# KyleVanMeter/MVOLPS

Hardware: AMD Instinct MI355X
Metric: simplex_pivots_per_s (higher is better)
Workload: dtype f64

## Files before the change

mvolps_amd/csrc/engine.cpp:

```cpp
#include <hip/hip_runtime.h>

#include <cmath>
#include <cstdio>
#include <cstdlib>
#include <cstring>
#include <atomic>
#include <map>
#include <mutex>
#include <tuple>
#include <unordered_map>
#include <vector>

#include "engine.hpp"

struct DevMatrix {
  int m0 = 0, n = 0, lda = 0;
  double *plain = nullptr, *packed = nullptr;
  int *len = nullptr;
  std::vector<const void *> rows;
  ~DevMatrix() {
    if (packed && packed != plain) (void)hipFree(packed);
    if (plain) (void)hipFree(plain);
    if (len) (void)hipFree(len);
  }
// ... 727 lines not shown
    P->nflag[j] = sflag ? sflag[j] : std_flag(P->ctype[j]);
    nlb[j] = P->clb[j];
    nub[j] = P->cub[j];
    xn[j] = nb_value(P->nflag[j], nlb[j], nub[j]);
    any_x = any_x || xn[j] != 0.0;
  }
  for (int i = 1; i <= m; i++) {
    P->bvar[i] = i;
    blb[i] = P->rlb[i];
    bub[i] = P->rub[i];
  }
  const size_t rows_per_chunk = std::max<size_t>(1, ((size_t)32 << 20) / ((size_t)ld * 8));
  double *bounce = nullptr;
  HIPCHECK(hipHostMalloc((void **)&bounce, rows_per_chunk * ld * 8));
  for (size_t r0 = 0; r0 <= (size_t)m; r0 += rows_per_chunk) {
    size_t r1 = std::min<size_t>((size_t)m + 1, r0 + rows_per_chunk);
    for (size_t i = r0; i < r1; i++) {
      double *row = bounce + (i - r0) * ld;
      std::memset(row, 0, (size_t)ld * 8);
      if (i == 0) {
        double z = P->c[0];
        for (int j = 1; j <= n; j++) {
          row[j] = P->c[j];
          if (xn[j] != 0.0) z = std::fma(P->c[j], xn[j], z);
        }
        row[0] = z;
      } else {
        const double *a = P->A[i]->data();
        std::memcpy(row + 1, a + 1, (size_t)n * 8);
        double acc = 0.0;
        if (any_x)
          for (int j = 1; j <= n; j++)
            if (xn[j] != 0.0) acc = std::fma(a[j], xn[j], acc);
        row[0] = acc;
      }
    }
    HIPCHECK(hipMemcpyAsync(P->d_T + r0 * ld, bounce, (r1 - r0) * ld * 8, hipMemcpyHostToDevice, sc.stream));
    HIPCHECK(hipStreamSynchronize(sc.stream));
  }
  HIPCHECK(hipHostFree(bounce));
  HIPCHECK(hipMemcpyAsync(P->d_bvar, P->bvar.data(), (size_t)(m + 1) * 4, hipMemcpyHostToDevice, sc.stream));
  HIPCHECK(hipMemcpyAsync(P->d_blb, blb.data(), (size_t)(m + 1) * 8, hipMemcpyHostToDevice, sc.stream));
  HIPCHECK(hipMemcpyAsync(P->d_bub, bub.data(), (size_t)(m + 1) * 8, hipMemcpyHostToDevice, sc.stream));
  std::vector<int> nv((size_t)ld, 0), nf((size_t)ld, MVX_NS);
  for (int j = 1; j <= n; j++) {
    nv[j] = P->nvar[j];
    nf[j] = P->nflag[j];
  }
  HIPCHECK(hipMemcpyAsync(P->d_nvar, nv.data(), (size_t)ld * 4, hipMemcpyHostToDevice, sc.stream));
  HIPCHECK(hipMemcpyAsync(P->d_nflag, nf.data(), (size_t)ld * 4, hipMemcpyHostToDevice, sc.stream));
  HIPCHECK(hipMemcpyAsync(P->d_nlb, nlb.data(), (size_t)ld * 8, hipMemcpyHostToDevice, sc.stream));
  HIPCHECK(hipMemcpyAsync(P->d_nub, nub.data(), (size_t)ld * 8, hipMemcpyHostToDevice, sc.stream));
  HIPCHECK(hipStreamSynchronize(sc.stream));
  rebuild_pos(P);
  P->pending.clear();
  P->valid = true;
  P->sol_fresh = false;
  P->fresh_rows = -1;
  P->status = MVX_UNDEF;
  return true;
}

static void flush_update_events(Context &c, size_t used) {
  for (size_t k = 0; k + 1 < used; k += 2) {
    float ms = 0.f;
    HIPCHECK(hipEventElapsedTime(&ms, c.ev_pool[k], c.ev_pool[k + 1]));
    c.prof_update_ms += ms;
    c.prof_update_n++;
  }
}

constexpr int PERSIST_HEAD_STRIDE_MAX = 4;
static std::atomic<int> g_persist_mode{-1};
static std::atomic<bool> g_persist_broken{false};
static std::atomic<long long> g_persist_launches{0}, g_persist_aborts{0};
struct PersistPlan {
  int cpw = 0, nw = 0;
  size_t lds = 0;
};
static bool persist_plan(Context &c, const mvx_prob *P, PersistPlan *pl) {
  if (g_persist_broken) return false;
  if (g_persist_mode < 0) {
    const char *e = std::getenv("MVX_PERSIST");
    g_persist_mode = (e && e[0] == '0') ? 0 : ((e && e[0] == '2') ? 2 : 1);
  }
  if (!g_persist_mode) return false;
  static int cus = 0;
  if (!cus) {
    hipDeviceProp_t prop;
    if (hipGetDeviceProperties(&prop, c.dev) != hipSuccess) return false;
    cus = prop.multiProcessorCount;
  }
  const int m = P->m, n = P->n;
  if ((long)(m + 1) * (n + 1) < 32768) return false;
  if (g_persist_mode < 2 && (long)(m + 1) * (n + 1) > 700000) return false;
  const int cpw = (n + cus - 1) / cus;
  if (cpw > persist_max_cpw()) return false;
  pl->cpw = cpw;
  pl->nw = (n + cpw - 1) / cpw;
  if (pl->nw > 256) return false;
  pl->lds = persist_lds_bytes(m, cpw);
  return pl->lds <= (size_t)150 * 1024;
}

static bool ensure_persist(Context &c, SolveCtx &sc, const mvx_prob *P, const PersistPlan &pl) {
  const int words = persist_slot_words(P->m_cap);
  if (!sc.d_pabort) {
    HIPCHECK(hipMalloc((void **)&sc.d_pabort, 1024));
    HIPCHECK(hipMemsetAsync(sc.d_pabort, 0, 1024, sc.stream));
    HIPCHECK(hipHostMalloc((void **)&sc.h_pabort, 1024));
    sc.h_pabort[0] = 0;
    HIPCHECK(hipMalloc((void **)&sc.d_pcand, (size_t)2 * 256 * PERSIST_HEAD_STRIDE_MAX * 8));
    HIPCHECK(hipMalloc((void **)&sc.d_pctl, sizeof(Ctl)));
  }
  if (words > sc.p_msg_words) {
    HIPCHECK(hipStreamSynchronize(sc.stream));
    if (sc.d_pmsg) HIPCHECK(hipFree(sc.d_pmsg));
    HIPCHECK(hipMalloc((void **)&sc.d_pmsg, (size_t)2 * 256 * words * 8));
    sc.p_msg_words = words;
  }
  if (P->ld > sc.p_pw_ld) {
    HIPCHECK(hipStreamSynchronize(sc.stream));
    if (sc.d_ppw) HIPCHECK(hipFree(sc.d_ppw));
    HIPCHECK(hipMalloc((void **)&sc.d_ppw, (size_t)2 * P->ld * 8));
    sc.p_pw_ld = P->ld;
  }
  if (sc.p_backup_bytes != P->slab_bytes) {
    if (sc.p_backup) slab_recycle(c, sc.p_backup, sc.p_backup_bytes);
    sc.p_backup = slab_alloc(c, P->slab_bytes);
    sc.p_backup_bytes = sc.p_backup ? P->slab_bytes : 0;
    if (!sc.p_backup) {
      (void)g_last_error.exchange(0);
      return false;
    }
  }
  (void)pl;
  return true;
}

struct SolveJob {
  mvx_prob *P = nullptr;
  SolveCtx *sc = nullptr;
  mvx_smcp parm;
  enum { MAIN, PHASE1, FINAL } mode = MAIN;
  int batch = 8, pb = 4;
  int done = D_RUN;
  bool try_fused = false;
  bool try_dfused = false;
  bool persist_queued = false;
  int seen_steps = 0, seen_pivots = 0, seen_bulk = 0;
  int chain = 1, chain0 = 1;
  bool resident = false;
  bool cluster = false;
  ChainArgs cargs{};
  size_t ev_used = 0;
  bool profiled = false;
  int rc = 0;
  Ctl snap;
};

static int pivot_budget(const mvx_prob *P, const mvx_smcp &parm) {
  return parm.it_lim >= 0 ? parm.it_lim : 200 * (P->m + P->n) + 100000;
}

static void stage_copy_async(SolveCtx &sc, const mvx_prob *P) {
  HIPCHECK(hipEventRecord(sc.ev_b, sc.stream));
  if (!sc.stage_zc) HIPCHECK(hipMemcpyAsync(sc.h_stage, sc.d_stage, stage_size(P->m_cap, P->ld), hipMemcpyDeviceToHost, sc.stream));
  if (sc.d_pabort) HIPCHECK(hipMemcpyAsync(sc.h_pabort, sc.d_pabort, 512, hipMemcpyDeviceToHost, sc.stream));
}

static bool dual_fused_worth_it(const mvx_prob *P) {
  static int mode = -1;
  if (mode < 0) {
    const char *e = std::getenv("MVX_DUAL_FUSED");
    mode = e ? std::atoi(e) : 1;
  }
  if (mode == 0) return false;
  if (mode >= 2) return true;
  const long entries = (long)(P->m + 1) * (P->n + 1);
  return entries >= 2000000 && entries < 12000000;
}

static void job_begin(Context &c, SolveJob &J) {
  mvx_prob *P = J.P;
  SolveCtx &sc = *J.sc;
  ensure_scratch(sc, P->m_cap, P->ld);
  Ctl *h = sc.h_ctl;
  fill_ctl(sc, P, h);
  h->tol_bnd = J.parm.tol_bnd;
  h->tol_dj = J.parm.tol_dj;
  h->tol_piv = J.parm.tol_piv;
  h->budget = pivot_budget(P, J.parm);
  take_edits(P, h);
  upload_ctl(sc);
  HIPCHECK(hipEventRecord(sc.ev_a, sc.stream));
  {
    ChainArgs &a = J.cargs;
    a.c = sc.d_ctl;
    a.T = P->d_T;
    a.blb = P->d_blb; a.bub = P->d_bub; a.nlb = P->d_nlb; a.nub = P->d_nub; a.nflag = P->d_nflag;
    a.betab = sc.d_betab;
    for (int k = 0; k < 2; k++) {
      a.pw[k] = sc.d_pw[k];
      a.drowk[k] = sc.d_drowk[k]; a.pwk[k] = sc.d_pwk[k]; a.nlbk[k] = sc.d_nlbk[k]; a.nubk[k] = sc.d_nubk[k]; a.nflagk[k] = sc.d_nflagk[k];
      a.betak[k] = sc.d_betak[k]; a.blbk[k] = sc.d_blbk[k]; a.bubk[k] = sc.d_bubk[k];
    }
    a.pp = sc.d_ppart; a.rp = sc.d_rpart; a.ppstride = sc.pp_stride; a.rpstride = sc.rp_stride;
    a.srow0 = sc.d_srowk[0]; a.colq0 = sc.d_colqk[0];
    a.sstride = sc.sk_stride; a.cstride = sc.ck_stride;
    a.m = P->m; a.n = P->n; a.ld = P->ld; a.mcap1 = P->m_cap + 1;
    a.ncb = chain_ncb(P->n); a.nrb = chain_nrb(P->m);
    a.tol_dj = h->tol_dj; a.tol_piv = h->tol_piv; a.tol_bnd = h->tol_bnd; a.sgn = h->sgn;
    a.stall_limit = h->stall_limit;
    a.zeros = sc.d_zeros;
    a.xg = sc.d_xg; a.xg_bytes = (int)XG_BYTES; a.xabort = sc.d_xabort;
    a.nw = chain_cluster_nw(P->m, P->n); a.kmax = 0; a.tagbase = 0; a.boot = 0;
  }
  J.cluster = J.resident && cluster_wanted() && chain_cluster_kmax(P->m, P->n) > 0;
  J.try_fused = !P->hint_dual;
  J.chain = J.chain0 = h->chain_max;
  J.try_dfused = P->hint_dual && dual_fused_worth_it(P);
  J.profiled = c.prof && J.sc == &c.main;
  if (J.parm.it_lim > 8 && J.try_fused) J.batch = std::min(J.parm.it_lim, 256);
}

static void job_enqueue(Context &c, SolveJob &J) {
  mvx_prob *P = J.P;
  SolveCtx &sc = *J.sc;
  const int m = P->m, n = P->n;
  J.ev_used = 0;
  if (J.mode == SolveJob::FINAL) {
    launch_export(sc.d_ctl, sc.d_stage, m, n, 1, sc.stream);
    stage_copy_async(sc, P);
    return;
  }
  if (J.mode == SolveJob::PHASE1) {
    for (int k = 0; k < J.pb; k++) {
      launch_p1_head(sc.d_ctl, sc.stream);
      launch_p1_fix(sc.d_ctl, n, sc.stream);
      launch_p1_select(sc.d_ctl, sc.stream);
      launch_update(sc.d_ctl, m + 1, n, sc.stream);
    }
    launch_export(sc.d_ctl, sc.d_stage, m, n, 0, sc.stream);
    stage_copy_async(sc, P);
    return;
  }
  const int batch = J.batch;
  if (J.profiled && c.ev_pool.size() < (size_t)2 * batch + 4) {
    size_t old = c.ev_pool.size();
    c.ev_pool.resize((size_t)2 * batch + 4);
    for (size_t k = old; k < c.ev_pool.size(); k++) HIPCHECK(hipEventCreate(&c.ev_pool[k]));
  }
  const int remaining = (J.parm.it_lim >= 0) ? std::max(0, J.parm.it_lim - J.seen_pivots) : (1 << 30);
  auto ev = [&]() {
    if (J.profiled) HIPCHECK(hipEventRecord(c.ev_pool[J.ev_used++], sc.stream));
  };
  int depth;
  if (J.try_fused) depth = std::max(0, std::min(batch, remaining));
  else depth = std::max(1, std::min(batch, remaining));
  auto body = [&](int m_grid) {
    if (J.try_fused) {
      PersistPlan pl;
      if (depth > 0 && !J.profiled && J.resident && !(J.cluster && !g_cluster_broken.load()) && persist_plan(c, P, &pl) && ensure_persist(c, sc, P, pl)) {
        launch_select(sc.d_ctl, sc.stream);
        launch_update(sc.d_ctl, m_grid, n, sc.stream, 1, 1);
        HIPCHECK(hipMemcpyAsync(sc.p_backup, P->slab, P->slab_bytes, hipMemcpyDeviceToDevice, sc.stream));
        HIPCHECK(hipMemcpyAsync(sc.d_pctl, sc.d_ctl, sizeof(Ctl), hipMemcpyDeviceToDevice, sc.stream));
        HIPCHECK(hipMemcpyAsync(sc.d_ppw, sc.d_pw[0], (size_t)P->ld * 8, hipMemcpyDeviceToDevice, sc.stream));
        HIPCHECK(hipMemcpyAsync(sc.d_ppw + P->ld, sc.d_pw[1], (size_t)P->ld * 8, hipMemcpyDeviceToDevice, sc.stream));
        const int head_stride = 4;
        HIPCHECK(hipMemsetAsync(sc.d_pcand, 0, (size_t)2 * pl.nw * head_stride * 8, sc.stream));
        const int steps = 1 << 24;
        if (launch_persist(sc.d_ctl, sc.d_pcand, sc.d_pmsg, sc.d_pabort, (unsigned long long *)(sc.d_pabort + 16), P->m, pl.cpw, pl.nw, sc.p_msg_words, steps, head_stride, sc.stream) == 0) {
          J.persist_queued = true;
          g_persist_launches++;
          launch_select(sc.d_ctl, sc.stream);
          launch_update(sc.d_ctl, m_grid, n, sc.stream, 1, 1);
        } else {
          g_persist_broken = true;
        }
      } else {
        const size_t e_generic = J.ev_used;
        if (J.profiled) J.ev_used += 2;
        if (depth > 0) {
          const bool cl = J.cluster && !g_cluster_broken.load();
          if (!cl) launch_pboot(J.cargs, sc.stream);
          bool first = true;
          const int kc = cl ? std::max(1, std::min(J.chain0, chain_cluster_kmax(m, n))) : std::max(1, J.chain);
          auto chain_launch = [&](int steps) {
            J.cargs.kmax = steps;
            J.cargs.boot = first ? 1 : 0;
            first = false;
            J.cargs.tagbase = sc.xtag;
            sc.xtag += 128;
            if (launch_chain(J.cargs, sc.stream) != 0) g_cluster_broken.store(true);
            g_cluster_launches++;
          };
          for (int left = depth; left > 0;) {
            const int steps = std::min(kc, left);
            if (cl) chain_launch(steps);
            else
              for (int t = 0; t < steps; t++) launch_pstep(J.cargs, t, sc.stream);
            ev();
            launch_fbc3(J.cargs, steps, sc.stream);
            ev();
            launch_fpatch(J.cargs, steps, sc.stream);
            left -= steps;
          }
          if (J.parm.it_lim >= 0 && depth >= remaining && !cl) launch_pc(J.cargs, 0, sc.stream);
        }
        launch_select(sc.d_ctl, sc.stream);
        if (J.profiled) HIPCHECK(hipEventRecord(c.ev_pool[e_generic], sc.stream));
        launch_update(sc.d_ctl, m_grid, n, sc.stream, 1, 1);
        if (J.profiled) HIPCHECK(hipEventRecord(c.ev_pool[e_generic + 1], sc.stream));
      }
    } else if (J.try_dfused) {
      launch_select(sc.d_ctl, sc.stream);
      launch_update(sc.d_ctl, m_grid, n, sc.stream, 1, 1);
      if (depth > 1) {
        launch_dboot(sc.d_ctl, n, sc.stream);
        launch_db(sc.d_ctl, m_grid, n, sc.stream);
        for (int k = 0; k < depth - 1; k++) {
          launch_da(sc.d_ctl, n, sc.stream);
          launch_db(sc.d_ctl, m_grid, n, sc.stream);
        }
      }
    } else {
      for (int k = 0; k < depth; k++) {
        launch_dsel(sc.d_ctl, m, n, sc.stream);
        launch_select(sc.d_ctl, sc.stream);
        ev();
        launch_update(sc.d_ctl, m_grid, n, sc.stream, 1, 1);
        ev();
      }
    }
    launch_export(sc.d_ctl, sc.d_stage, m_grid, n, 0, sc.stream);
    stage_copy_async(sc, P);
  };
  body(m);
}

static bool job_finalize(SolveJob &J) {
  mvx_prob *P = J.P;
  SolveCtx &sc = *J.sc;
  const Ctl &snap = J.snap;
  const unsigned char *s = sc.h_stage;
  const double *beta = (const double *)(s + sizeof(Ctl));
  const double *dj = beta + (P->m_cap + 1);
  const int *bv = (const int *)(dj + P->ld);
  const int *nv = bv + (P->m_cap + 1);
  const int *nf = nv + P->ld;
  P->beta.assign(beta, beta + P->m + 1);
  P->dj.assign(dj, dj + P->n + 1);
  P->bvar.assign(bv, bv + P->m + 1);
  P->nvar.assign(nv, nv + P->n + 1);
  P->nflag.assign(nf, nf + P->n + 1);
  rebuild_pos(P);
  P->sol_fresh = true;
  P->fresh_rows = -1;
  float ms = 0.f;
  HIPCHECK(hipEventElapsedTime(&ms, sc.ev_a, sc.ev_b));
  P->last_ms = ms;
  P->it_cnt += snap.it_cnt;
  P->bland_cnt += snap.n_bland;
  P->pert_cnt += snap.n_pert;
  P->hint_dual = false;
  switch (J.done) {
    case D_OPT: P->status = MVX_OPT; J.rc = 0; break;
    case D_UNBND: P->status = MVX_UNBND; J.rc = 0; break;
    case D_NOFEAS: P->status = MVX_NOFEAS; J.rc = 0; break;
    case D_ITLIM:
      P->status = (snap.phase == PH_PRIMAL2) ? MVX_FEAS : MVX_INFEAS;
      J.rc = MVX_EITLIM;
      break;
    default: P->status = MVX_UNDEF; J.rc = MVX_EFAIL; break;
  }
  return true;
}

static bool job_collect(Context &c, SolveJob &J) {
  SolveCtx &sc = *J.sc;
  Ctl &snap = J.snap;
  if (J.persist_queued) {
    J.persist_queued = false;
    if (sc.h_pabort[0]) {
      mvx_prob *P = J.P;
      g_persist_broken = true;
      g_persist_aborts++;
      std::fprintf(stderr, "mvx: resident-tableau launch aborted (workgroups not co-resident in time); using the two-kernel path from now on\n");
      HIPCHECK(hipMemcpyAsync(P->slab, sc.p_backup, P->slab_bytes, hipMemcpyDeviceToDevice, sc.stream));
      HIPCHECK(hipMemcpyAsync(sc.d_ctl, sc.d_pctl, sizeof(Ctl), hipMemcpyDeviceToDevice, sc.stream));
      HIPCHECK(hipMemcpyAsync(sc.d_pw[0], sc.d_ppw, (size_t)P->ld * 8, hipMemcpyDeviceToDevice, sc.stream));
      HIPCHECK(hipMemcpyAsync(sc.d_pw[1], sc.d_ppw + P->ld, (size_t)P->ld * 8, hipMemcpyDeviceToDevice, sc.stream));
      HIPCHECK(hipMemsetAsync(sc.d_pabort, 0, sizeof(int), sc.stream));
      sc.h_pabort[0] = 0;
      J.try_fused = true;
      return false;
    }
  }
  std::memcpy(&snap, sc.h_stage, sizeof(Ctl));
  if (J.mode == SolveJob::FINAL) return job_finalize(J);
  if (J.mode == SolveJob::PHASE1) {
    if (snap.done == D_RUN) {
      J.pb = std::min(J.pb * 2, 64);
      return false;
    }
    if (snap.done == D_PFEAS) {
      snap.rounds++;
      if (snap.rounds >= 64) {
        J.done = D_FAIL;
        J.mode = SolveJob::FINAL;
        return false;
      }
      snap.done = D_RUN;
      snap.phase = PH_START;
      *sc.h_ctl = snap;
      upload_ctl(sc);
      J.mode = SolveJob::MAIN;
      J.batch = 8;
      J.try_fused = false;
      J.try_dfused = false;
      return false;
    }
    J.done = snap.done;
    return job_finalize(J);
  }
  if (J.profiled) {
    const int steps_now = snap.n_bulk;
    flush_update_events(c, std::min(J.ev_used, (size_t)2 * (size_t)(steps_now - J.seen_steps)));
    J.seen_steps = steps_now;
  }
  if (snap.cl_abort) {
    g_cluster_broken.store(true);
    g_cluster_aborts++;
    std::fprintf(stderr, "mvx: cluster selection launch aborted (peer workgroups not reachable in time); using two launches per chained step from now on\n");
    HIPCHECK(hipMemsetAsync(sc.d_xabort, 0, sizeof(int), sc.stream));
  }
  J.done = snap.done;
  {
    const int dp = snap.it_cnt - J.seen_pivots, db = snap.n_bulk - J.seen_bulk;
    if (J.chain0 > 1 && db >= 4) {
      if (2 * dp < J.chain * db) J.chain = std::max(1, J.chain / 2);
      else if (10 * dp >= 9 * J.chain * db) J.chain = std::min(J.chain0, J.chain * 2);
    }
    J.seen_bulk = snap.n_bulk;
  }
  J.seen_pivots = snap.it_cnt;
  J.try_fused = (snap.phase == PH_PRIMAL2) && snap.stall < snap.stall_limit;
  J.try_dfused = (snap.phase == PH_DUAL) && snap.stall < snap.stall_limit && dual_fused_worth_it(J.P);
  if (J.done == D_NEED_PHASE1) {
    snap.done = D_RUN;
    snap.phase = PH_PHASE1;
    snap.p1_init = 1;
    snap.p1_fix_q = 0;
    *sc.h_ctl = snap;
    upload_ctl(sc);
    J.mode = SolveJob::PHASE1;
    J.pb = 4;
    return false;
  }
  if (J.done != D_RUN) return job_finalize(J);
  J.batch = std::min(J.batch * 2, 256);
  return false;
}

static bool already_solved(const mvx_prob *P, const mvx_smcp &parm) {
  if (!P->valid || parm.it_lim == 0) return false;
  if (P->status != MVX_OPT) return false;
  return P->last_tol[0] == parm.tol_bnd && P->last_tol[1] == parm.tol_dj && P->last_tol[2] == parm.tol_piv;
}
static void remember_tolerances(mvx_prob *P, const mvx_smcp &parm) {
  P->last_tol[0] = parm.tol_bnd;
  P->last_tol[1] = parm.tol_dj;
  P->last_tol[2] = parm.tol_piv;
}

static bool job_prepare(SolveJob &J, mvx_prob *P, const mvx_smcp *parm) {
  J.P = P;
  if (parm) J.parm = *parm;
  else mvx_init_smcp(&J.parm);
  if (P->m < 1 || P->n < 1) {
    P->status = MVX_UNDEF;
    J.rc = MVX_EFAIL;
    return false;
  }
  if (already_solved(P, J.parm)) {
    P->last_ms = 0.0;
    J.rc = 0;
    return false;
  }
  if (!P->valid && !build_slack_tableau(P)) {
    J.rc = MVX_EFAIL;
    return false;
  }
  remember_tolerances(P, J.parm);
  return true;
}

static int solve_once(mvx_prob *P, const mvx_smcp *parm, bool aux) {
  SolveJob J;
  if (!job_prepare(J, P, parm)) return J.rc;
  P->fresh_rows = -1;
  Context &c = ctx();
  HIPCHECK(hipSetDevice(c.dev));
  std::unique_lock<std::recursive_mutex> main_lock(c.main_mu);
  flush_copies(c);
  if (aux) main_lock.unlock();
  std::unique_lock<std::mutex> aux_lock(c.aux_mu, std::defer_lock);
  if (aux) aux_lock.lock();
  if (aux && !c.aux_ready) {
    init_solve_ctx(c.aux);
    c.aux_ready = true;
  }
  J.sc = aux ? &c.aux : &c.main;
  static std::atomic<bool> g_resident_token{false};
  bool expected = false;
  J.resident = g_resident_token.compare_exchange_strong(expected, true);
  job_begin(c, J);
  for (;;) {
    job_enqueue(c, J);
    HIPCHECK(hipStreamSynchronize(J.sc->stream));
    if (job_collect(c, J)) break;
  }
  if (J.resident) g_resident_token.store(false);
  return J.rc;
}

static int g_check_every = 1024;
static double g_refresh_tol = 1e-9;
void set_refresh(int check_every, double tol) {
  g_check_every = check_every > 0 ? check_every : 1024;
  g_refresh_tol = tol >= 0.0 ? tol : 1e-9;
}

constexpr int REFRESH_SAMPLE_ROWS = 32;
static double row_residual_sample(const mvx_prob *P, int rows);
double row_residual(const mvx_prob *P) { return row_residual_sample(P, 0); }

static double row_residual_sample(const mvx_prob *P, int rows) {
  if (!P->valid) return 0.0;
  refresh_solution(P);
  const int m = P->m, n = P->n;
  auto value = [&](int k) {
    const int pos = P->pos[(size_t)k];
    if (pos > 0) return P->beta[(size_t)pos];
    double lb, ub;
    var_bounds(P, k, &lb, &ub);
    return nb_value(P->nflag[(size_t)-pos], lb, ub);
  };
  std::vector<double> x((size_t)n + 1, 0.0);
  for (int j = 1; j <= n; j++) x[(size_t)j] = value(m + j);
  double worst = 0.0;
  const bool all = rows <= 0 || rows >= m;
  const int cnt = all ? m : rows;
  for (int k = 0; k < cnt; k++) {
    const int i = all ? k + 1 : 1 + (int)(((unsigned)P->it_cnt * 2654435761u + (unsigned)k * 0x9E3779B1u) % (unsigned)m);
    const double *a = P->A[(size_t)i]->data();
    double acc = 0.0;
    for (int j = 1; j <= n; j++) acc = acc + a[j] * x[(size_t)j];
    const double xr = value(i);
    const double r = std::fabs(acc - xr) / (1.0 + std::fabs(xr));
    if (r > worst) worst = r;
  }
  return worst;
}

static bool refresh_tableau(mvx_prob *P) {
  Context &c = ctx();
  MAIN_LOCK(c);
  flush_copies(c);
  SolveCtx &sc = c.main;
  const int m = P->m, n = P->n;
  std::vector<int> tflag((size_t)m + n + 1, 0), sflag((size_t)n + 1, 0);
  for (int j = 1; j <= n; j++) tflag[(size_t)P->nvar[(size_t)j]] = P->nflag[(size_t)j];
  for (int j = 1; j <= n; j++) sflag[(size_t)j] = tflag[(size_t)m + j] ? tflag[(size_t)m + j] : std_flag(P->ctype[(size_t)j]);
  const int status = P->status;
  if (!build_slack_tableau(P, sflag.data())) return false;
  ensure_scratch(sc, P->m_cap, P->ld);
  HIPCHECK(hipMemcpyAsync(sc.d_tflag, tflag.data(), tflag.size() * 4, hipMemcpyHostToDevice, sc.stream));
  fill_ctl(sc, P, sc.h_ctl);
  upload_ctl(sc);
  for (int k = m + 1; k <= m + n; k++) {
    if (tflag[(size_t)k]) continue;
    launch_refresh_select(sc.d_ctl, sc.d_tflag, k, sc.stream);
    launch_update(sc.d_ctl, m, n, sc.stream);
// ... 942 lines not shown
```

mvolps_amd/csrc/kernels.hip:

```cpp
#include <hip/hip_runtime.h>

#include <cmath>
#include <cstdlib>

#include "mvx_internal.hpp"

namespace mvx {

#define TIDX ((int)threadIdx.x)

__device__ __forceinline__ double xdiv(double a, double b) {
  const double q = a / b;
  const double aq = fabs(q);
  if (!(aq > 1e-290 && aq < 1e290)) return q;
  const double r = fma(-q, b, a);
  if (r == 0.0) return q;
  const bool up = (r > 0.0) == (b > 0.0);
  long long bits = __double_as_longlong(q);
  bits += ((q > 0.0) == up) ? 1 : -1;
  const double q1 = __longlong_as_double(bits);
  const double r1 = fma(-q1, b, a);
  return (fabs(r1) < fabs(r)) ? q1 : q;
}

// ... 2048 lines not shown
    tf = ubq - lbq;
    if (p == 0 || tf <= tstep) flip = true;
  }
  if (!flip && p == 0) {
    if (lead && g == 0) c->fstate = F_STOP;
    return;
  }
  PR_STAMP(1);
  const int pr = flip ? 1 : p;
  const double val0 = T[(size_t)pr * ld + jc];
  const double piv = A.colq0[(size_t)g * A.cstride + pr];
  const double bp = (g == 0) ? A.betab[pr] : A.betak[xr][pr];
  const double plb = (g == 0) ? A.blb[pr] : A.blbk[xr][pr], pub = (g == 0) ? A.bub[pr] : A.bubk[xr][pr];
  const double rcp = A.colq0[(size_t)rl * A.cstride + pr];
  rec.ip = xdiv(1.0, rec.piv);
  const double rcd = xdiv(rcp, rec.piv);
  PR_STAMP(2);
  double sj = 0.0, dnew, wnew;
  int fnew, kind, lf = 0, stall_new;
  double delta = 0.0, bound = 0.0, s0 = 0.0, xq = 0.0;
  if (flip) {
    const int nf = (sdir > 0) ? MVX_NU : MVX_NL;
    delta = (sdir > 0) ? tf : -tf;
    kind = ST_FLIP;
    lf = nf;
    dnew = (j == 0) ? fma(dq, delta, dj) : dj;
    wnew = wj;
    fnew = (j == q) ? nf : fj;
    stall_new = 0;
  } else {
    double val = val0;
#define PR_ROWSTEP(S, TV)                                                                              \
  if ((S) < g) {                                                                                       \
    const int lk = rl_i(rec.kind, (S));                                                                \
    if (lk == ST_PIVOT) {                                                                              \
      const int lp = rl_i(rec.p, (S)), lq = rl_i(rec.q, (S));                                          \
      if (lp == p) val = (j == lq) ? rl_d(rec.ip, (S)) : -(TV);                                        \
      else val = (j == lq) ? rl_d(rcd, (S)) : fma(-rl_d(rcp, (S)), (TV), val);                         \
    }                                                                                                  \
  }
#pragma unroll
    for (int s = 0; s < 16; s++) { PR_ROWSTEP(s, ta[s]) }
    if (g > 16) {
#pragma unroll
      for (int s = 0; s < 16; s++) { PR_ROWSTEP(16 + s, tb[s]) }
    }
#undef PR_ROWSTEP
    bound = p_up ? pub : plb;
    lf = dev_leave_flag(plb, pub, p_up);
    s0 = xdiv(bp - bound, piv);
    sj = (j == 0) ? s0 : xdiv(val, piv);
    dnew = (j == q) ? xdiv(dq, piv) : fma(-dq, sj, dj);
    if (j == q) {
      const double cc = xdiv(wq, piv * piv);
      wnew = cc > 1.0 ? cc : 1.0;
      lbj = plb;
      ubj = pub;
    } else {
      const double cc = sj * sj * wq;
      wnew = cc > wj ? cc : wj;
    }
    fnew = (j == q) ? lf : fj;
    kind = ST_PIVOT;
    xq = dev_nb_value(fq, lbq, ubq);
    stall_new = (tstep <= DEGEN_TOL) ? stall + 1 : 0;
  }
  if (!act || j == 0) fnew = MVX_NS;
  PR_STAMP(3);
  Cand best{0.0, 0.0, 0, 0};
  if (fnew != MVX_NS) {
    Cand x{0.0, 0.0, 0, 0};
    if (price_col(fnew, A.sgn * dnew, A.tol_dj, j, wnew, x)) best = x;
  }
  publish_pricing(A, best, b, dnew, wnew, lbj, ubj, fnew, s_slots, s_pay);
  PR_STAMP(4);
  if (act) {
    A.srow0[(size_t)g * A.sstride + j] = sj;
    A.drowk[xw][j] = dnew;
    A.pwk[xw][j] = (j >= 1) ? wnew : 1.0;
    A.nflagk[xw][j] = (j >= 1) ? fnew : MVX_NS;
    A.nlbk[xw][j] = lbj;
    A.nubk[xw][j] = ubj;
  }
  if (lead) {
    c->ch_kind[g] = kind;
    c->ch_p[g] = flip ? 0 : p;
    c->ch_q[g] = q;
    c->ch_lf[g] = lf;
    c->ch_piv[g] = flip ? 1.0 : piv;
    c->ch_xq[g] = xq;
    c->ch_s0[g] = s0;
    c->ch_delta[g] = delta;
    c->ch_elb[g] = lbq;
    c->ch_eub[g] = ubq;
    c->ch_llb[g] = plb;
    c->ch_lub[g] = pub;
    c->ch_bound[g] = bound;
    c->ch_pup[g] = p_up;
    c->ch_stall[g] = stall_new;
    c->ch_cnt[g] = used + (flip ? 0 : 1);
    c->ch_ok[g] = epoch;
    c->pc_n = g + 1;
  }
  PR_STAMP(5);
#undef PR_STAMP
}

constexpr int XNW = 64;
constexpr int XNF = 8;
enum : int { XAUX_SC0 = 1, XAUX_SC1 = 16 };
typedef unsigned xu4 __attribute__((ext_vector_type(4)));

struct XCtx {
  __amdgpu_buffer_rsrc_t rs;
  int w, nw;
  unsigned tag;
  int xno;
  int *xabort;
  bool dead;
  bool flag;
};

__device__ __forceinline__ double ld_sc1(const double *p) {
  return __longlong_as_double((long long)__hip_atomic_load(reinterpret_cast<const unsigned long long *>(p), __ATOMIC_RELAXED, __HIP_MEMORY_SCOPE_AGENT));
}

template <int MODE, int NP>
__device__ __forceinline__ Cand xchg(XCtx &X, Cand mine, const double (&pin)[NP], double (&pout)[NP], Cand (*s_slots)[4], double (*s_pay)[4][5]) {
  const int lane = TIDX & 63, wave = TIDX >> 6, b = X.xno & 1;
  int ol;
  Cand wb = wave_argbest<MODE>(mine, &ol);
  wb.aux = (wb.aux & 0xffff) | (__ballot(X.flag) ? 0x10000 : 0);
  if (lane == 0) s_slots[b][wave] = wb;
#pragma unroll
  for (int k = 0; k < NP; k++) {
    const double v = rl_d(pin[k], ol);
    if (lane == 0) s_pay[b][wave][k] = v;
  }
  __syncthreads();
  Cand bb = s_slots[b][0];
  int bw = 0, fl = bb.aux & 0x10000;
#pragma unroll
  for (int k = 1; k < 4; k++) {
    const Cand y = s_slots[b][k];
    fl |= y.aux & 0x10000;
    if (cand_better<MODE>(y, bb)) {
      bb = y;
      bw = k;
    }
  }
  bb.aux = (bb.aux & 0xffff) | fl;
  const unsigned tag = X.tag;
  const unsigned reg = (unsigned)(X.xno & 3) * (unsigned)(XNF * XNW * 16);
  if (TIDX < 3 + NP) {
    double v;
    if (TIDX == 0) v = bb.k1;
    else if (TIDX == 1) v = bb.k2;
    else if (TIDX == 2) v = __hiloint2double(bb.aux, bb.idx);
    else v = s_pay[b][bw][TIDX - 3];
    const xu4 x = {(unsigned)__double2loint(v), tag, (unsigned)__double2hiint(v), tag};
    __builtin_amdgcn_raw_buffer_store_b128(x, X.rs, reg + (unsigned)(TIDX * XNW + X.w) * 16, 0, XAUX_SC0);
  }
  double rec[3 + NP];
  const int lr = lane < X.nw ? lane : 0;
  unsigned spins = 0;
  for (;;) {
    bool ok = true;
#pragma unroll
    for (int f = 0; f < 3 + NP; f++) {
      const xu4 x = __builtin_amdgcn_raw_buffer_load_b128(X.rs, reg + (unsigned)(f * XNW + lr) * 16, 0, XAUX_SC1);
      ok &= (x.y == tag) & (x.w == tag);
      rec[f] = __hiloint2double((int)x.z, (int)x.x);
    }
    if (__all(ok)) break;
    ++spins;
    if ((spins & 255u) == 0) {
      if (spins > 2000000u) __hip_atomic_store(X.xabort, 1, __ATOMIC_RELAXED, __HIP_MEMORY_SCOPE_AGENT);
      if (spins > 2000000u || __hip_atomic_load(X.xabort, __ATOMIC_RELAXED, __HIP_MEMORY_SCOPE_AGENT)) {
        X.dead = true;
        break;
      }
    }
    __builtin_amdgcn_s_sleep(1);
  }
  X.tag++;
  X.xno++;
  Cand rc{0.0, 0.0, 0, 0};
  if (lane < X.nw && !X.dead) rc = Cand{rec[0], rec[1], __double2loint(rec[2]), __double2hiint(rec[2])};
  int wl;
  Cand win = wave_argbest<MODE>(rc, &wl);
  X.flag = __ballot((rc.aux & 0x10000) != 0) != 0ull;
  win.aux = (int)(short)(win.aux & 0xffff);
#pragma unroll
  for (int k = 0; k < NP; k++) pout[k] = rl_d(rec[3 + k], wl);
  return win;
}

template <int CPT, int RPT>
__global__ __launch_bounds__(256) void k_chain(const ChainArgs A) {
  extern __shared__ double hist[];
  __shared__ Cand s_slots[2][4];
  __shared__ double s_pay[2][4][5];
  __shared__ int s_kind[KCH], s_p[KCH], s_q[KCH];
  __shared__ double s_piv[KCH], s_ip[KCH], s_wv[4][2][KCH];
  if (blockIdx.x & 7) return;
  const int w = (int)blockIdx.x >> 3, t = TIDX, lane = t & 63, wave = t >> 6;
  Ctl *const c = A.c;
  const int nw = A.nw, TT = nw * 256, gt = w * 256 + t;
  const int m = A.m, n = A.n, kmax = A.kmax;
  const size_t ld = (size_t)A.ld;
  const double *const T = A.T;
  const bool lead = (gt == 0);
  unsigned long long *const dbg = c->dbg;
#define CH_STAMP(K) do { if (dbg && lead) dbg[(size_t)g * 16 + (K)] = __builtin_amdgcn_s_memrealtime(); } while (0)
  const int done = c->done, fstate0 = c->fstate, budget = c->budget, perturbed = c->perturbed, aborted = c->cl_abort, epoch = c->pc_epoch;
  const int phase0 = c->phase, n_edits = c->n_edits, cur0 = c->curA & 1;
  int stall = c->stall;
  const bool boot = (A.boot != 0);
  const bool fresh = boot && (phase0 == PH_START);
  const int fstate = boot ? F_RUN : fstate0;
  const bool boot_off = boot && (stall >= A.stall_limit || !(phase0 == PH_PRIMAL2 || (fresh && n_edits == 0)));
  double d[CPT], wgt[CPT], lbj[CPT], ubj[CPT], sqn[CPT];
  int f[CPT], jj[CPT];
#pragma unroll
  for (int u = 0; u < CPT; u++) {
    const int j = 1 + gt + u * TT;
    const bool act = (j <= n);
    const int jc = act ? j : n;
    jj[u] = j;
    d[u] = T[jc];
    wgt[u] = fresh ? 1.0 : A.pw[boot ? cur0 : 0][jc];
    f[u] = act ? A.nflag[jc] : MVX_NS;
    lbj[u] = A.nlb[jc];
    ubj[u] = A.nub[jc];
    sqn[u] = 0.0;
  }
  double z = T[0];
  double be[RPT], lb[RPT], ub[RPT];
  int ii[RPT];
#pragma unroll
  for (int u = 0; u < RPT; u++) {
    const int i = 1 + gt + u * TT;
    const int ic = (i <= m) ? i : m;
    ii[u] = i;
    be[u] = boot ? T[(size_t)ic * ld] : A.betab[ic];
    lb[u] = A.blb[ic];
    ub[u] = A.bub[ic];
  }
  if (done != D_RUN || fstate != F_RUN || aborted) return;
  if (boot_off) {
    if (lead) c->fstate = F_OFF;
    return;
  }
  XCtx X;
  X.rs = __builtin_amdgcn_make_buffer_rsrc(A.xg, 0, A.xg_bytes, 0x00027000);
  X.w = w;
  X.nw = nw;
  X.tag = A.tagbase + 1;
  X.xno = 0;
  X.xabort = A.xabort;
  X.dead = false;
  X.flag = false;
  if (fresh) {
    const double tolb = A.tol_bnd;
#pragma unroll
    for (int u = 0; u < RPT; u++) {
      if (ii[u] <= m) {
        if (lb[u] > -INFINITY && be[u] < lb[u] - tolb * (1.0 + fabs(lb[u]))) X.flag = true;
        if (ub[u] < INFINITY && be[u] > ub[u] + tolb * (1.0 + fabs(ub[u]))) X.flag = true;
      }
    }
  }
#define HS(S, U) hist[((size_t)(S) * (CPT + RPT) + (U)) * 256 + t]
#define HC(S, U) hist[((size_t)(S) * (CPT + RPT) + CPT + (U)) * 256 + t]
  int g = 0, used = 0;
  Cand pc;
  double pp[5], po[5];
#define PRICE()                                                                                          \
  do {                                                                                                   \
    pc = Cand{0.0, 0.0, 0, 0};                                                                           \
    pp[0] = d[0]; pp[1] = wgt[0]; pp[2] = lbj[0]; pp[3] = ubj[0]; pp[4] = sqn[0];                        \
    _Pragma("unroll") for (int u = 0; u < CPT; u++) {                                                    \
      Cand x{0.0, 0.0, 0, 0};                                                                            \
      if (f[u] != MVX_NS && price_col(f[u], A.sgn * d[u], A.tol_dj, jj[u], wgt[u], x) && cand_better<0>(x, pc)) { \
        pc = x;                                                                                          \
        pc.aux = (x.aux > 0 ? 1 : 0) | (f[u] << 1);                                                      \
        pp[0] = d[u]; pp[1] = wgt[u]; pp[2] = lbj[u]; pp[3] = ubj[u]; pp[4] = sqn[u];                    \
      }                                                                                                  \
    }                                                                                                    \
  } while (0)
  PRICE();
  Cand qc = xchg<0, 5>(X, pc, pp, po, s_slots, s_pay);
  if (boot && !X.dead) {
    if (X.flag) {
      if (lead) c->fstate = F_OFF;
      return;
    }
    if (lead) {
      c->fstate = F_RUN;
      c->step = ST_NONE;
    }
  }
  X.flag = false;
  bool end_itlim = false;
  for (;;) {
    if (X.dead) break;
    const int q = qc.idx;
    const bool none = (q == 0);
    const int left = (budget < 0) ? 1 : budget - used;
    if (none || left <= 0 || stall >= A.stall_limit) {
      const bool itlim = (!none && left <= 0 && stall < A.stall_limit && !perturbed);
      if (g == 0) {
        if (lead) {
          c->fstate = F_STOP;
          c->phase = PH_PRIMAL2;
          if (itlim) {
            c->done = D_ITLIM;
            c->step = ST_NONE;
          }
        }
      } else
        end_itlim = itlim;
      break;
    }
    if (g >= kmax) break;
    CH_STAMP(0);
    const int sdir = (qc.aux & 1) ? 1 : -1, fq = qc.aux >> 1;
    const double dq = po[0], wq = po[1], lbq = po[2], ubq = po[3];
    double a[RPT];
#pragma unroll
    for (int u = 0; u < RPT; u++) a[u] = T[(size_t)((ii[u] <= m) ? ii[u] : m) * ld + q];
    {
      double sqv = po[4];
      if (lane < g - 1) sqv = ld_sc1(A.srow0 + (size_t)lane * A.sstride + q);
      if (lane < g) s_wv[wave][0][lane] = sqv;
    }
    const int gu = __builtin_amdgcn_readfirstlane(g);
    const bool ispc = (lane < gu) && (s_kind[lane < KCH ? lane : 0] == ST_PIVOT);
    const unsigned pivm = (unsigned)__ballot(ispc);
    const unsigned spc = (unsigned)__ballot(ispc && s_q[lane < KCH ? lane : 0] == q);
    {
      int s0 = 0;
#define COL_BLOCK(N)                                                                                                     \
  if (gu - s0 >= N) {                                                                                                    \
    const unsigned bm = ((1u << N) - 1u) << s0;                                                                          \
    double hc8[RPT][N], sq8[N];                                                                                          \
    int lp8[N];                                                                                                          \
    _Pragma("unroll") for (int k = 0; k < N; k++) {                                                                      \
      sq8[k] = s_wv[wave][0][s0 + k];                                                                                    \
      lp8[k] = s_p[s0 + k];                                                                                              \
      _Pragma("unroll") for (int u = 0; u < RPT; u++) hc8[u][k] = HC(s0 + k, u);                                         \
    }                                                                                                                    \
    if ((pivm & bm) == bm && (spc & bm) == 0u) {                                                                         \
      _Pragma("unroll") for (int k = 0; k < N; k++) {                                                                    \
        _Pragma("unroll") for (int u = 0; u < RPT; u++) a[u] = (ii[u] == lp8[k]) ? -sq8[k] : fma(-hc8[u][k], sq8[k], a[u]); \
      }                                                                                                                  \
    } else {                                                                                                             \
      _Pragma("unroll") for (int k = 0; k < N; k++) {                                                                    \
        const int sx = s0 + k;                                                                                           \
        if ((pivm >> sx) & 1u) {                                                                                         \
          if ((spc >> sx) & 1u) {                                                                                        \
            const double ips = s_ip[sx], pvs = s_piv[sx];                                                                \
            _Pragma("unroll") for (int u = 0; u < RPT; u++) a[u] = (ii[u] == lp8[k]) ? ips : xdiv(hc8[u][k], pvs);       \
          } else {                                                                                                       \
            _Pragma("unroll") for (int u = 0; u < RPT; u++) a[u] = (ii[u] == lp8[k]) ? -sq8[k] : fma(-hc8[u][k], sq8[k], a[u]); \
          }                                                                                                              \
        }                                                                                                                \
      }                                                                                                                  \
    }                                                                                                                    \
    s0 += N;                                                                                                             \
  }
      while (gu - s0 >= 8) { COL_BLOCK(8) }
      COL_BLOCK(4)
      COL_BLOCK(2)
      COL_BLOCK(1)
#undef COL_BLOCK
    }
    CH_STAMP(1);
    Cand rb{0.0, 0.0, 0, 0};
    double rp[4] = {a[0], be[0], lb[0], ub[0]}, ro[4];
#pragma unroll
    for (int u = 0; u < RPT; u++) {
      Cand x{0.0, 0.0, 0, 0};
      if (ii[u] <= m) {
        A.colq0[(size_t)g * A.cstride + ii[u]] = a[u];
        if (ratio_row(a[u], sdir, be[u], lb[u], ub[u], 0, A.tol_piv, ii[u], x) && cand_better<1>(x, rb)) {
          rb = x;
          rp[0] = a[u]; rp[1] = be[u]; rp[2] = lb[u]; rp[3] = ub[u];
        }
      }
      HC(g, u) = a[u];
    }
    CH_STAMP(2);
    const Cand pw = xchg<1, 4>(X, rb, rp, ro, s_slots, s_pay);
    if (X.dead) break;
    CH_STAMP(3);
    const int p = pw.idx, p_up = pw.aux;
    const double tstep = pw.k1, piv = ro[0], bp = ro[1], plb = ro[2], pub = ro[3];
    double val[CPT];
#pragma unroll
    for (int u = 0; u < CPT; u++) val[u] = T[(size_t)p * ld + ((jj[u] <= n) ? jj[u] : n)];
    double rcp_l = 0.0;
    if (lane < g) rcp_l = ld_sc1(A.colq0 + (size_t)lane * A.cstride + p);
    bool flip = false;
    double tf = 0.0;
    if (lbq > -INFINITY && ubq < INFINITY && fq != MVX_NF) {
      tf = ubq - lbq;
      if (p == 0 || tf <= tstep) flip = true;
    }
    if (!flip && p == 0) {
      if (lead && g == 0) {
        c->fstate = F_STOP;
        c->phase = PH_PRIMAL2;
      }
      break;
    }
    int kind, lf, stall_new;
    double delta = 0.0, bound = 0.0, s0 = 0.0, xq = 0.0, ip = 1.0;
    if (flip) {
      kind = ST_FLIP;
      lf = (sdir > 0) ? MVX_NU : MVX_NL;
      delta = (sdir > 0) ? tf : -tf;
      stall_new = 0;
#pragma unroll
      for (int u = 0; u < RPT; u++) be[u] = fma(a[u], delta, be[u]);
      z = fma(dq, delta, z);
#pragma unroll
      for (int u = 0; u < CPT; u++) {
        if (jj[u] == q) f[u] = lf;
        sqn[u] = 0.0;
      }
    } else {
      kind = ST_PIVOT;
      bound = p_up ? pub : plb;
      lf = dev_leave_flag(plb, pub, p_up);
      s0 = xdiv(bp - bound, piv);
      xq = dev_nb_value(fq, lbq, ubq);
      ip = xdiv(1.0, piv);
      stall_new = (tstep <= DEGEN_TOL) ? stall + 1 : 0;
#pragma unroll
      for (int u = 0; u < RPT; u++) {
        if (ii[u] == p) {
          be[u] = xq - s0;
          lb[u] = lbq;
          ub[u] = ubq;
        } else
          be[u] = fma(-a[u], s0, be[u]);
      }
      CH_STAMP(4);
      if (lane < g) {
        const double rcp = rcp_l;
        s_wv[wave][0][lane] = rcp;
        s_wv[wave][1][lane] = xdiv(rcp, s_piv[lane]);
      }
      const unsigned spr = (unsigned)__ballot(ispc && s_p[lane < KCH ? lane : 0] == p);
      {
        int s0 = 0;
#define ROW_BLOCK(N)                                                                                                     \
  if (gu - s0 >= N) {                                                                                                    \
    const unsigned bm = ((1u << N) - 1u) << s0;                                                                          \
    double hs8[CPT][N], cp8[N], cd8[N];                                                                                  \
    int lq8[N];                                                                                                          \
    _Pragma("unroll") for (int k = 0; k < N; k++) {                                                                      \
      cp8[k] = s_wv[wave][0][s0 + k];                                                                                    \
      cd8[k] = s_wv[wave][1][s0 + k];                                                                                    \
      lq8[k] = s_q[s0 + k];                                                                                              \
      _Pragma("unroll") for (int u = 0; u < CPT; u++) hs8[u][k] = HS(s0 + k, u);                                         \
    }                                                                                                                    \
    if ((pivm & bm) == bm && (spr & bm) == 0u) {                                                                         \
      _Pragma("unroll") for (int k = 0; k < N; k++) {                                                                    \
        _Pragma("unroll") for (int u = 0; u < CPT; u++) val[u] = (jj[u] == lq8[k]) ? cd8[k] : fma(-cp8[k], hs8[u][k], val[u]); \
      }                                                                                                                  \
    } else {                                                                                                             \
      _Pragma("unroll") for (int k = 0; k < N; k++) {                                                                    \
        const int sx = s0 + k;                                                                                           \
        if ((pivm >> sx) & 1u) {                                                                                         \
          if ((spr >> sx) & 1u) {                                                                                        \
            const double ips = s_ip[sx];                                                                                 \
            _Pragma("unroll") for (int u = 0; u < CPT; u++) val[u] = (jj[u] == lq8[k]) ? ips : -hs8[u][k];               \
          } else {                                                                                                       \
            _Pragma("unroll") for (int u = 0; u < CPT; u++) val[u] = (jj[u] == lq8[k]) ? cd8[k] : fma(-cp8[k], hs8[u][k], val[u]); \
          }                                                                                                              \
        }                                                                                                                \
      }                                                                                                                  \
    }                                                                                                                    \
    s0 += N;                                                                                                             \
  }
        while (gu - s0 >= 8) { ROW_BLOCK(8) }
        ROW_BLOCK(4)
        ROW_BLOCK(2)
        ROW_BLOCK(1)
#undef ROW_BLOCK
      }
      CH_STAMP(5);
#pragma unroll
      for (int u = 0; u < CPT; u++) {
        const int j = jj[u];
        const double sj = xdiv(val[u], piv);
        if (j == q) {
          d[u] = xdiv(dq, piv);
          const double cc = xdiv(wq, piv * piv);
          wgt[u] = cc > 1.0 ? cc : 1.0;
          lbj[u] = plb;
          ubj[u] = pub;
          f[u] = lf;
        } else {
          d[u] = fma(-dq, sj, d[u]);
          const double cc = sj * sj * wq;
          wgt[u] = cc > wgt[u] ? cc : wgt[u];
        }
        if (j <= n) A.srow0[(size_t)g * A.sstride + j] = sj;
        HS(g, u) = sj;
        sqn[u] = sj;
      }
      z = fma(-dq, s0, z);
      if (lead) A.srow0[(size_t)g * A.sstride] = s0;
    }
    s_kind[g] = kind;
    s_p[g] = flip ? 0 : p;
    s_q[g] = q;
    s_piv[g] = flip ? 1.0 : piv;
    s_ip[g] = ip;
    used += flip ? 0 : 1;
    if (lead) {
      c->ch_kind[g] = kind;
      c->ch_p[g] = flip ? 0 : p;
      c->ch_q[g] = q;
      c->ch_lf[g] = lf;
      c->ch_piv[g] = flip ? 1.0 : piv;
      c->ch_xq[g] = xq;
      c->ch_s0[g] = s0;
      c->ch_delta[g] = delta;
      c->ch_elb[g] = lbq;
      c->ch_eub[g] = ubq;
      c->ch_llb[g] = plb;
      c->ch_lub[g] = pub;
      c->ch_bound[g] = bound;
      c->ch_pup[g] = p_up;
      c->ch_stall[g] = stall_new;
      c->ch_cnt[g] = used;
      c->ch_ok[g] = epoch;
    }
    CH_STAMP(6);
    PRICE();
    CH_STAMP(7);
    stall = stall_new;
    g++;
    qc = xchg<0, 5>(X, pc, pp, po, s_slots, s_pay);
    if (dbg && lead) dbg[(size_t)(g - 1) * 16 + 8] = __builtin_amdgcn_s_memrealtime();
  }
#undef PRICE
#undef CH_STAMP
#undef HS
#undef HC
  if (X.dead) {
    if (lead) {
      c->pc_n = 0;
      c->cl_abort = 1;
    }
    return;
  }
  if (g == 0 && fresh) {
#pragma unroll
    for (int u = 0; u < CPT; u++) {
      if (jj[u] <= n) {
        A.pw[0][jj[u]] = 1.0;
        A.pw[1][jj[u]] = 1.0;
      }
    }
  }
  if (g > 0) {
    const int xf = g & 1;
#pragma unroll
    for (int u = 0; u < CPT; u++) {
      if (jj[u] <= n) {
        A.drowk[xf][jj[u]] = d[u];
        A.pwk[xf][jj[u]] = wgt[u];
      }
    }
    if (lead) {
      A.drowk[xf][0] = z;
      A.pwk[xf][0] = 1.0;
    }
  }
  if (lead) {
    c->pc_n = g;
    if (g > 0) {
      c->phase = PH_PRIMAL2;
      c->pc_itlim = end_itlim ? 1 : 0;
    }
  }
}

__device__ void chain_commit(const ChainArgs &A, Ctl *c, int nch) {
  __shared__ int s_cp[KCH], s_cq[KCH], s_ck[KCH], s_rf[KCH], s_cf[KCH], s_R[KCH], s_C[KCH];
  const int t = TIDX;
  const bool on = (t < nch);
  int kind = 0, p = 0, q = 0;
  if (on) {
    kind = c->ch_kind[t];
    p = c->ch_p[t];
    q = c->ch_q[t];
    s_ck[t] = kind;
    s_cp[t] = p;
    s_cq[t] = q;
    s_R[t] = (kind == ST_PIVOT) ? c->bvar[p] : 0;
    s_C[t] = (kind == ST_PIVOT) ? c->nvar[q] : 0;
  }
  __syncthreads();
  bool lastrow = true, lastcol = true, lastflag = true;
  if (on) {
    int rf = t, cf = t;
    for (int u = t - 1; u >= 0; u--) {
      if (s_ck[u] != ST_PIVOT) continue;
      if (s_cp[u] == p) rf = u;
      if (s_cq[u] == q) cf = u;
    }
    s_rf[t] = rf;
    s_cf[t] = cf;
    for (int u = t + 1; u < nch; u++) {
      if (s_cq[u] == q) lastflag = false;
      if (s_ck[u] != ST_PIVOT) continue;
      if (s_cp[u] == p) lastrow = false;
      if (s_cq[u] == q) lastcol = false;
// ... 1097 lines not shown
```

Baseline: 58280.

## Shrink cluster exchange record and skip per-element pivot-index selects in chained updates

The cross-workgroup candidate exchange now sends one fewer 16-byte field per wave. The secondary key is dropped and, in mode 1, rebuilt from the absolute value of the first payload entry. In the chained column and row update loops, the per-element compare-and-select against the pivot row or column index is moved behind a wave-uniform ballot mask. The mask records whether any lane of the wave owns that index, so most steps run plain FMAs. The host also logs the cluster-abort handling once per job instead of on every snapshot. The risks are that the rebuilt secondary key must match the original one for mode 1, and the hit-mask range check must cover every owned index.

```diff
diff --git a/mvolps_amd/csrc/engine.cpp b/mvolps_amd/csrc/engine.cpp
--- a/mvolps_amd/csrc/engine.cpp
+++ b/mvolps_amd/csrc/engine.cpp
@@ -903,6 +903,7 @@
   int chain = 1, chain0 = 1;
   bool resident = false;
   bool cluster = false;
+  bool cl_abort_seen = false;
   ChainArgs cargs{};
   size_t ev_used = 0;
   bool profiled = false;
@@ -1181,7 +1182,8 @@
     flush_update_events(c, std::min(J.ev_used, (size_t)2 * (size_t)(steps_now - J.seen_steps)));
     J.seen_steps = steps_now;
   }
-  if (snap.cl_abort) {
+  if (snap.cl_abort && !J.cl_abort_seen) {
+    J.cl_abort_seen = true;
     g_cluster_broken.store(true);
     g_cluster_aborts++;
     std::fprintf(stderr, "mvx: cluster selection launch aborted (peer workgroups not reachable in time); using two launches per chained step from now on\n");
diff --git a/mvolps_amd/csrc/kernels.hip b/mvolps_amd/csrc/kernels.hip
--- a/mvolps_amd/csrc/kernels.hip
+++ b/mvolps_amd/csrc/kernels.hip
@@ -2224,22 +2224,21 @@
   bb.aux = (bb.aux & 0xffff) | fl;
   const unsigned tag = X.tag;
   const unsigned reg = (unsigned)(X.xno & 3) * (unsigned)(XNF * XNW * 16);
-  if (TIDX < 3 + NP) {
+  if (TIDX < 2 + NP) {
     double v;
     if (TIDX == 0) v = bb.k1;
-    else if (TIDX == 1) v = bb.k2;
-    else if (TIDX == 2) v = __hiloint2double(bb.aux, bb.idx);
-    else v = s_pay[b][bw][TIDX - 3];
+    else if (TIDX == 1) v = __hiloint2double(bb.aux, bb.idx);
+    else v = s_pay[b][bw][TIDX - 2];
     const xu4 x = {(unsigned)__double2loint(v), tag, (unsigned)__double2hiint(v), tag};
     __builtin_amdgcn_raw_buffer_store_b128(x, X.rs, reg + (unsigned)(TIDX * XNW + X.w) * 16, 0, XAUX_SC0);
   }
-  double rec[3 + NP];
+  double rec[2 + NP];
   const int lr = lane < X.nw ? lane : 0;
   unsigned spins = 0;
   for (;;) {
     bool ok = true;
 #pragma unroll
-    for (int f = 0; f < 3 + NP; f++) {
+    for (int f = 0; f < 2 + NP; f++) {
       const xu4 x = __builtin_amdgcn_raw_buffer_load_b128(X.rs, reg + (unsigned)(f * XNW + lr) * 16, 0, XAUX_SC1);
       ok &= (x.y == tag) & (x.w == tag);
       rec[f] = __hiloint2double((int)x.z, (int)x.x);
@@ -2258,13 +2257,13 @@
   X.tag++;
   X.xno++;
   Cand rc{0.0, 0.0, 0, 0};
-  if (lane < X.nw && !X.dead) rc = Cand{rec[0], rec[1], __double2loint(rec[2]), __double2hiint(rec[2])};
+  if (lane < X.nw && !X.dead) rc = Cand{rec[0], MODE == 1 ? fabs(rec[2]) : 0.0, __double2loint(rec[1]), __double2hiint(rec[1])};
   int wl;
   Cand win = wave_argbest<MODE>(rc, &wl);
   X.flag = __ballot((rc.aux & 0x10000) != 0) != 0ull;
   win.aux = (int)(short)(win.aux & 0xffff);
 #pragma unroll
-  for (int k = 0; k < NP; k++) pout[k] = rl_d(rec[3 + k], wl);
+  for (int k = 0; k < NP; k++) pout[k] = rl_d(rec[2 + k], wl);
   return win;
 }
 
@@ -2411,6 +2410,20 @@
     const bool ispc = (lane < gu) && (s_kind[lane < KCH ? lane : 0] == ST_PIVOT);
     const unsigned pivm = (unsigned)__ballot(ispc);
     const unsigned spc = (unsigned)__ballot(ispc && s_q[lane < KCH ? lane : 0] == q);
+    const int wb = 1 + w * 256 + wave * 64;
+    unsigned hitc, hitr;
+    {
+      const int sl = lane < KCH ? lane : 0;
+      const int lp = s_p[sl], lq = s_q[sl];
+      bool hp = false, hq = false;
+#pragma unroll
+      for (int u = 0; u < (RPT > CPT ? RPT : CPT); u++) {
+        if (u < RPT) hp |= (unsigned)(lp - (wb + u * TT)) < 64u;
+        if (u < CPT) hq |= (unsigned)(lq - (wb + u * TT)) < 64u;
+      }
+      hitc = (unsigned)__ballot(lane < gu && hp);
+      hitr = (unsigned)__ballot(lane < gu && hq);
+    }
     {
       int s0 = 0;
 #define COL_BLOCK(N)                                                                                                     \
@@ -2425,7 +2438,11 @@
     }                                                                                                                    \
     if ((pivm & bm) == bm && (spc & bm) == 0u) {                                                                         \
       _Pragma("unroll") for (int k = 0; k < N; k++) {                                                                    \
-        _Pragma("unroll") for (int u = 0; u < RPT; u++) a[u] = (ii[u] == lp8[k]) ? -sq8[k] : fma(-hc8[u][k], sq8[k], a[u]); \
+        _Pragma("unroll") for (int u = 0; u < RPT; u++) a[u] = fma(-hc8[u][k], sq8[k], a[u]);                           \
+        if (__builtin_expect((hitc >> (s0 + k)) & 1u, 0)) {              \
+          asm volatile("");                                                                                              \
+          _Pragma("unroll") for (int u = 0; u < RPT; u++) a[u] = (ii[u] == lp8[k]) ? -sq8[k] : a[u];                      \
+        }                                                                                                                \
       }                                                                                                                  \
     } else {                                                                                                             \
       _Pragma("unroll") for (int k = 0; k < N; k++) {                                                                    \
@@ -2541,7 +2558,11 @@
     }                                                                                                                    \
     if ((pivm & bm) == bm && (spr & bm) == 0u) {                                                                         \
       _Pragma("unroll") for (int k = 0; k < N; k++) {                                                                    \
-        _Pragma("unroll") for (int u = 0; u < CPT; u++) val[u] = (jj[u] == lq8[k]) ? cd8[k] : fma(-cp8[k], hs8[u][k], val[u]); \
+        _Pragma("unroll") for (int u = 0; u < CPT; u++) val[u] = fma(-cp8[k], hs8[u][k], val[u]);                        \
+        if (__builtin_expect((hitr >> (s0 + k)) & 1u, 0)) {                                                                                   \
+          asm volatile("");                                                                                              \
+          _Pragma("unroll") for (int u = 0; u < CPT; u++) val[u] = (jj[u] == lq8[k]) ? cd8[k] : val[u];                   \
+        }                                                                                                                \
       }                                                                                                                  \
     } else {                                                                                                             \
       _Pragma("unroll") for (int k = 0; k < N; k++) {                                                                    \
```

New measurement: 58860, median of 6. Within noise of the previous version (+1.0%).
